# Etschbeijer/GibbsSampling

Hardware: NVIDIA B200
Metric: gibbs_window_scores_per_sec (higher is better)
Workload: dtype f64

## Files before the change

### gibbssampling_b200/csrc/gibbs_cluster.cuh

```cuda
#pragma once
#include "gibbs_kernels.cuh"

namespace gibbs {

constexpr int CL_T = 16;

__device__ __forceinline__ uint32_t cluster_ctarank() {
    uint32_t r;
    asm volatile("mov.u32 %0, %%cluster_ctarank;" : "=r"(r));
    return r;
}
__device__ __forceinline__ void cluster_barrier() {
    asm volatile("barrier.cluster.arrive.release.aligned;\n\tbarrier.cluster.wait.acquire.aligned;" ::: "memory");
}
__device__ __forceinline__ uint32_t map_to_rank(const void *smem_ptr, uint32_t rank) {
    uint32_t out;
    asm volatile("mapa.shared::cluster.u32 %0, %1, %2;" : "=r"(out) : "r"(smem_u32(smem_ptr)), "r"(rank));
    return out;
}
__device__ __forceinline__ void st_cluster_u32(uint32_t addr, uint32_t v) {
    asm volatile("st.shared::cluster.u32 [%0], %1;" ::"r"(addr), "r"(v) : "memory");
}
__device__ __forceinline__ void st_cluster_u64(uint32_t addr, uint64_t v) {
    asm volatile("st.shared::cluster.u64 [%0], %1;" ::"r"(addr), "l"(v) : "memory");
}
__device__ __forceinline__ void cp_async16(void *dst, const void *src) {
    asm volatile("cp.async.cg.shared.global [%0], [%1], 16;" ::"r"(smem_u32(dst)), "l"(src) : "memory");
}
__device__ __forceinline__ void cp_async_wait_all() { asm volatile("cp.async.commit_group;\n\tcp.async.wait_group 0;" ::: "memory"); }

template <int C>
__host__ __device__ constexpr int cl_flags_off() { return 704; }
template <int C>
__host__ __device__ constexpr int cl_delta_off() { return cl_flags_off<C>() + 2 * C * CL_T * 4; }
template <int C>
__host__ __device__ constexpr int cl_ctl_off() { return cl_delta_off<C>() + 2 * C * CL_T * 16; }
template <int C>
__host__ __device__ constexpr int cl_tables_off() { return (cl_ctl_off<C>() + 16 + 63) / 64 * 64; }
template <int C>
__host__ __device__ inline size_t cluster_smem_bytes(int n, int row_words) {
    return (size_t)cl_tables_off<C>() + (size_t)CL_T * WARP_TABLE_BYTES + (size_t)CL_T * 2 * row_words * 4 + (size_t)n * 4 * sizeof(WEnt);
}

template <int KP, int C>
static __global__ void __launch_bounds__(32 * CL_T, 1) chain_cluster_kernel(const ChainArgs a) {
    extern __shared__ __align__(128) unsigned char smem_raw[];
    constexpr int T = CL_T, THREADS = 32 * CL_T, GW = C * CL_T;
    const int tid = threadIdx.x, lane = tid & 31, warp = tid >> 5;
    const uint32_t crank = cluster_ctarank();
    const int gw = (int)crank * T + warp;
    const int entry = blockIdx.x / C;
    if (entry >= *a.pending_in_n) return;
    const int chain = a.pending_in[entry];

    const int N = a.s.n, k = a.k, row_words = a.s.row_words;
    int32_t *total = reinterpret_cast<int32_t *>(smem_raw);
    int32_t *fix = reinterpret_cast<int32_t *>(smem_raw + 512);
    uint32_t *lut = reinterpret_cast<uint32_t *>(smem_raw + 640);
    int32_t *flags = reinterpret_cast<int32_t *>(smem_raw + cl_flags_off<C>());
    uint64_t *delta = reinterpret_cast<uint64_t *>(smem_raw + cl_delta_off<C>());
    int32_t *ctl = reinterpret_cast<int32_t *>(smem_raw + cl_ctl_off<C>());
    WarpTables WT;
    {
        unsigned char *b = smem_raw + cl_tables_off<C>() + warp * WARP_TABLE_BYTES;
        WT.wcol = reinterpret_cast<double *>(b);
        WT.ptab = reinterpret_cast<int32_t *>(b + 1024);
        WT.lgcol = reinterpret_cast<int32_t *>(b + 2048);
        WT.counts = reinterpret_cast<int32_t *>(b + 2560);
    }
    require_aligned_tables(WT);
    uint32_t *rows = reinterpret_cast<uint32_t *>(smem_raw + cl_tables_off<C>() + T * WARP_TABLE_BYTES) + warp * 2 * row_words;
    WEnt *wtab_s = reinterpret_cast<WEnt *>(smem_raw + cl_tables_off<C>() + T * WARP_TABLE_BYTES + (size_t)T * 2 * row_words * 4);

    int32_t *sites = a.sites + (size_t)chain * N;
    double *hv = a.hv + (size_t)chain * N;
    double *scores = a.scores + (size_t)chain * N;

    if (tid < 16) lut[tid] = hist_lut_entry(tid);
    {
        const int4 *src = reinterpret_cast<const int4 *>(a.wtab);
        int4 *dst = reinterpret_cast<int4 *>(wtab_s);
        for (int i = tid; i < N * 4; i += THREADS) dst[i] = __ldg(src + i);
    }
    uint32_t r_flag = 0, r_delta = 0;
    if (lane < C) {
        r_flag = map_to_rank(flags + gw, (uint32_t)lane);
        r_delta = map_to_rank(delta + 2 * gw, (uint32_t)lane);
    }
    __syncthreads();
    cluster_barrier();

    unsigned long long st_updates = 0, st_windows = 0, st_slow = 0, st_spec = 0;
    int st_sweeps = 0, capped = 0;
    int phase, sweeps_in_phase;
    {
        const int r = a.resume[chain];
        phase = r & 127;
        capped = (r >> 7) & 1;
        sweeps_in_phase = r >> 8;
    }
    bool resumed = true, paused = false;
    const int ulen = a.s.uniform_len;

    auto fetch_row = [&](int seq, int slot) {
        const uint4 *src = reinterpret_cast<const uint4 *>(a.s.packed + (size_t)seq * row_words);
        uint4 *dst = reinterpret_cast<uint4 *>(rows + slot * row_words);
        for (int i = lane; i < (row_words >> 2); i += 32) cp_async16(dst + i, src + i);
    };

    while (phase != PH_DONE) {
        const int mode = phase == PH_LEFT ? SHIFT_LEFT : phase == PH_RIGHT ? SHIFT_RIGHT : SHIFT_NONE;
        if (phase == PH_LEFT || phase == PH_RIGHT || (phase == PH_GREEDY && (sweeps_in_phase == 0 || resumed)))
            site_counts<KP, T>(a.s, sites, -1, k, mode, total, lut, fix, tid);
        resumed = false;
        bool changed = false;
        int n0 = 0;
        int width = (phase == PH_GREEDY) ? max(1, min(GW, a.min_width)) : GW;
        unsigned round = 0;
        int have = -1, have_slot = 0;
        int pf_n = -1, pf_site = 0, pf_len = 0;
        double pf_hv = 0.0;
        {
            const int n = n0 + gw;
            if (n < N) {
                fetch_row(n, 0);
                have = n;
                have_slot = 0;
                pf_n = n;
                pf_site = __ldcg(sites + n);
                pf_hv = __ldcg(hv + n);
                pf_len = ulen > 0 ? ulen : __ldg(a.s.len + n);
            }
        }
        while (n0 < N) {
            const int n = n0 + gw;
            const bool active = n < N && gw < width;
            int flag = 0, w = 0, Wn = 0;
            double p = 0.0;
            uint64_t own = 0, neu = 0;
            const int n_pred = n + GW;
            if (n < N) {
                if (have != n) {
                    cp_async_wait_all();
                    __syncwarp();
                    fetch_row(n, have_slot);
                    have = n;
                }
                cp_async_wait_all();
                __syncwarp();
            }
            const int cur_slot = have_slot;
            int nx_site = 0, nx_len = 0;
            double nx_hv = 0.0;
            if (n_pred < N) {
                fetch_row(n_pred, cur_slot ^ 1);
                nx_site = __ldcg(sites + n_pred);
                nx_hv = __ldcg(hv + n_pred);
                nx_len = ulen > 0 ? ulen : __ldg(a.s.len + n_pred);
            }
            int site_n = 0;
            if (active) {
                const uint32_t *row = rows + cur_slot * row_words;
                int len_n;
                double hv_n;
                if (pf_n == n) {
                    site_n = pf_site;
                    hv_n = pf_hv;
                    len_n = pf_len;
                } else {
                    site_n = __ldcg(sites + n);
                    hv_n = __ldcg(hv + n);
                    len_n = ulen > 0 ? ulen : __ldg(a.s.len + n);
                }
                Wn = len_n - k + 1;
                own = kmer_shared<KP>(row, shifted_site(site_n, len_n, k, mode));
                build_tables_impl<KP, false, true>(WT, total, true, own, k, wtab_s, lane, 0);
                const bool slow = pick_argmax<KP>(WT, row, Wn, k, a.fast_ok, lane, p, w);
                const bool accept = score_improves(p, hv_n, hv_n != hv_n ? __ldcg(scores + n) : 0.0);
                const bool moved = accept && (w != site_n);
                if (moved && phase == PH_GREEDY) neu = kmer_shared<KP>(row, w);
                flag = (accept ? 1 : 0) | (moved ? 2 : 0) | (slow ? 4 : 0) | 8;
            }
            const uint32_t par = (round & 1u);
            ++round;
            if (lane < C) {
                if ((flag & 2) && phase == PH_GREEDY) {
                    st_cluster_u64(r_delta + par * GW * 16, own);
                    st_cluster_u64(r_delta + par * GW * 16 + 8, neu);
                }
                st_cluster_u32(r_flag + par * GW * 4, (uint32_t)flag);
            }
            cluster_barrier();
            const int32_t *fl = flags + par * GW;
            unsigned movers_lo = __ballot_sync(FULL, lane < GW && (fl[lane < GW ? lane : 0] & 2) != 0);
            unsigned movers_hi[(GW + 31) / 32] = {};
            movers_hi[0] = movers_lo;
#pragma unroll
            for (int q = 1; q < (GW + 31) / 32; ++q) movers_hi[q] = __ballot_sync(FULL, (fl[q * 32 + lane] & 2) != 0);
            int first_mover = GW;
            bool any_moved = false;
#pragma unroll
            for (int q = (GW + 31) / 32 - 1; q >= 0; --q)
                if (movers_hi[q]) {
                    any_moved = true;
                    first_mover = q * 32 + __ffs(movers_hi[q]) - 1;
                }
            if (phase != PH_GREEDY) first_mover = GW;
            const int last_commit = min(first_mover, width - 1);
            changed |= any_moved;
            if (active) {
                if (gw <= last_commit) {
                    st_updates += 1;
                    st_windows += (unsigned long long)Wn;
                    st_slow += (flag & 4) ? 1 : 0;
                    if ((flag & 1) && lane == 0) {
                        sites[n] = w;
                        hv[n] = p;
                    }
                } else {
                    st_spec += 1;
                }
            }
            const int committed = min(last_commit + 1, N - n0);
            n0 += committed;
            if (phase == PH_GREEDY) {
                if (first_mover < GW) {
                    if (warp == 0 && lane < k) {
                        const uint64_t o = delta[(par * GW + first_mover) * 2], nw = delta[(par * GW + first_mover) * 2 + 1];
                        const int bo = (int)((o >> (2 * lane)) & 3u), bn = (int)((nw >> (2 * lane)) & 3u);
                        if (bo != bn) {
                            total[lane * 4 + bo] -= 1;
                            total[lane * 4 + bn] += 1;
                        }
                    }
                    __syncthreads();
                    width = max(max(1, min(GW, a.min_width)), width >> 1);
                } else {
                    width = min(GW, width * 2);
                }
            }
            if (n_pred < N) {
                if (committed == GW) {
                    have = n_pred;
                    have_slot = cur_slot ^ 1;
                    pf_n = n_pred;
                    pf_site = nx_site;
                    pf_hv = nx_hv;
                    pf_len = nx_len;
                } else {
                    have = -2;
                    have_slot = cur_slot;
                    pf_n = -1;
                }
            } else {
                have = -2;
                have_slot = cur_slot;
                pf_n = -1;
            }
        }
        cp_async_wait_all();
        __syncwarp();
        st_sweeps += 1;
        ++sweeps_in_phase;
        bool next = !changed;
        if (!next && sweeps_in_phase >= a.max_sweeps) {
            next = true;
            capped = 1;
        }
        if (next) {
            sweeps_in_phase = 0;
            phase = next_phase(phase + 1, a.phase_mask);
        }
        int want_pause = 0;
        if (phase != PH_DONE && a.pause_below > 0 && crank == 0 && tid == 0)
            want_pause = (*(volatile int32_t *)a.active <= a.pause_below) ? 1 : 0;
// ... 41 lines not shown
```

### gibbssampling_b200/csrc/gibbs_device.cuh

```cuda
#pragma once
#include <cuda_runtime.h>
#include <stdint.h>
#include <type_traits>

namespace gibbs {

constexpr unsigned FULL = 0xffffffffu;
constexpr int LG_FRAC_BITS = 11;
constexpr int KEY_IDX_BITS = 8;
constexpr int MAX_COLS = 32;
constexpr double LN2 = 0.6931471805599453;

enum ShiftMode { SHIFT_NONE = 0, SHIFT_LEFT = 1, SHIFT_RIGHT = 2 };
enum StatSlot { ST_SITE_UPDATES = 0, ST_WINDOW_SCORES = 1, ST_SWEEPS = 2, ST_EXACT_RESCANS = 3, ST_CAPPED = 4,
                ST_SPECULATED = 5, ST_NSLOTS = 8 };

struct __align__(16) WEnt {
    double w;
    int32_t lg;
    int32_t pad;
};

struct DeviceSeqs {
    const uint32_t *packed;
// ... 328 lines not shown
                        if (2 * p + 1 < k) dst[e1] += v1;
                    } else {
                        atomicAdd(&dst[e0], v0);
                        if (2 * p + 1 < k) atomicAdd(&dst[e1], v1);
                    }
                }
            }
            lo[p] = hi[p] = 0;
        }
    }
};

template <int KP>
struct KmerCounter {
    static constexpr int NW = (KP > 8) ? 2 : 1;
    static constexpr bool HI4 = (KP == 9 || KP == 10);
    using Word = typename std::conditional<(KP > 8), uint64_t, uint32_t>::type;
    uint32_t nib[HI4 ? 1 : NW][3][2];
    uint32_t byt[NW][3][2][2];
    uint32_t hq[HI4 ? 3 : 1];
    int quads;
    __device__ __forceinline__ void clear() {
#pragma unroll
        for (int w = 0; w < NW; ++w)
#pragma unroll
            for (int b = 0; b < 3; ++b)
#pragma unroll
                for (int p = 0; p < 2; ++p) {
                    if (!HI4 || w == 0) nib[HI4 ? 0 : w][b][p] = 0;
                    byt[w][b][p][0] = byt[w][b][p][1] = 0;
                }
        if (HI4) hq[0] = hq[1] = hq[2] = 0;
        quads = 0;
    }
    __device__ __forceinline__ void spill() {
#pragma unroll
        for (int w = 0; w < NW; ++w)
#pragma unroll
            for (int b = 0; b < 3; ++b)
#pragma unroll
                for (int p = 0; p < 2; ++p) {
                    uint32_t v;
                    if (HI4 && w == 1) {
                        v = (p == 0 ? hq[b] : (hq[b] >> 2)) & 0x33333333u;
                    } else {
                        v = nib[HI4 ? 0 : w][b][p];
                        nib[HI4 ? 0 : w][b][p] = 0;
                    }
                    byt[w][b][p][0] += v & 0x0F0F0F0Fu;
                    byt[w][b][p][1] += (v >> 4) & 0x0F0F0F0Fu;
                }
        if (HI4) hq[0] = hq[1] = hq[2] = 0;
        quads = 0;
    }
    __device__ __forceinline__ void add4(const Word x[4]) {
        if (quads == 3) spill();
#pragma unroll
        for (int w = 0; w < (HI4 ? 1 : NW); ++w) {
            uint32_t f[4][3];
#pragma unroll
            for (int i = 0; i < 4; ++i) {
                const uint32_t v = (uint32_t)(x[i] >> (32 * w)), t = v >> 1;
                f[i][0] = v & ~t & 0x55555555u;
                f[i][1] = ~v & t & 0x55555555u;
                f[i][2] = v & t & 0x55555555u;
            }
#pragma unroll
            for (int b = 0; b < 3; ++b) {
                const uint32_t s3 = f[0][b] + f[1][b] + f[2][b];
                nib[w][b][0] += (s3 & 0x33333333u) + (f[3][b] & 0x11111111u);
                nib[w][b][1] += ((s3 >> 2) & 0x33333333u) + ((f[3][b] >> 2) & 0x11111111u);
            }
        }
        if constexpr (HI4) {
            const uint32_t h01 = __byte_perm((uint32_t)((uint64_t)x[0] >> 32), (uint32_t)((uint64_t)x[1] >> 32), 0x0040);
            const uint32_t h23 = __byte_perm((uint32_t)((uint64_t)x[2] >> 32), (uint32_t)((uint64_t)x[3] >> 32), 0x0040);
            const uint32_t v = __byte_perm(h01, h23, 0x5410), t = v >> 1;
            hq[0] += v & ~t & 0x55555555u;
            hq[1] += ~v & t & 0x55555555u;
            hq[2] += v & t & 0x55555555u;
        }
        ++quads;
    }
    __device__ __forceinline__ void flush(int32_t *dst, int k, int added, bool first, int lane) {
        spill();
        uint32_t mine[NW] = {};
#pragma unroll
        for (int w = 0; w < NW; ++w)
#pragma unroll
            for (int b = 0; b < 3; ++b)
#pragma unroll
                for (int p = 0; p < 2; ++p)
#pragma unroll
                    for (int h = 0; h < 2; ++h)
#pragma unroll
                        for (int g = 0; g < 2; ++g) {
                            const int it = (((b * 2 + p) * 2 + h) * 2 + g);
                            const int col0 = (HI4 && w == 1) ? 16 + 2 * h + p : 16 * w + 4 * g + 2 * h + p;
                            if (col0 < 2 * KP) {
                                const uint32_t s = __reduce_add_sync(FULL, (byt[w][b][p][h] >> (8 * g)) & 0x00FF00FFu);
                                if (lane == it) mine[w] = s;
                            }
                        }
        {
            const int g = lane & 1, h = (lane >> 1) & 1, p = (lane >> 2) & 1, b = lane >> 3;
#pragma unroll
            for (int w = 0; w < NW; ++w) {
                const int32_t v0 = (int32_t)(mine[w] & 0xFFFFu), v1 = (int32_t)(mine[w] >> 16);
                if (HI4 && w == 1) {
                    const int32_t half = v0 + v1, tot = half + __shfl_xor_sync(FULL, half, 1);
                    const int c = 16 + 2 * h + p;
                    if (lane < 24 && g == 0 && c < k) dst[c * 4 + b + 1] = first ? tot : dst[c * 4 + b + 1] + tot;
                } else if (lane < 24) {
                    const int c0 = 16 * w + 4 * g + 2 * h + p, c1 = c0 + 8;
                    if (c0 < k) dst[c0 * 4 + b + 1] = first ? v0 : dst[c0 * 4 + b + 1] + v0;
                    if (c1 < k) dst[c1 * 4 + b + 1] = first ? v1 : dst[c1 * 4 + b + 1] + v1;
                }
            }
        }
#pragma unroll
        for (int w = 0; w < NW; ++w)
#pragma unroll
            for (int b = 0; b < 3; ++b)
#pragma unroll
                for (int p = 0; p < 2; ++p) byt[w][b][p][0] = byt[w][b][p][1] = 0;
        if (lane < k) dst[lane * 4] = first ? added : dst[lane * 4] + added;
        __syncwarp();
    }
    static __device__ __forceinline__ void finish(int32_t *dst, int k, int lane) {
        if (lane < k) dst[lane * 4] -= dst[lane * 4 + 1] + dst[lane * 4 + 2] + dst[lane * 4 + 3];
        __syncwarp();
    }
};

template <int KP, bool SROWS>
__device__ __forceinline__ typename KmerCounter<KP>::Word gather_kmer(const uint32_t *__restrict__ rows, int row_words, int i, int pos) {
    uint32_t w0, w1, w2 = 0;
    if (SROWS) {
        const uint32_t *p = rows + (i * row_words + (pos >> 4));
        w0 = p[0];
        w1 = p[1];
        if (KP > 8) w2 = p[2];
    } else {
        const uint32_t *p = rows + (size_t)i * row_words + (pos >> 4);
        w0 = __ldg(p);
        w1 = __ldg(p + 1);
        if (KP > 8) w2 = __ldg(p + 2);
    }
    const uint32_t lo = __funnelshift_r(w0, w1, 2 * pos);
    if constexpr (KP > 8) {
        return ((uint64_t)__funnelshift_r(w1, w2, 2 * pos) << 32) | lo;
    } else {
        return lo;
    }
}
template <int KP>
__device__ __forceinline__ typename KmerCounter<KP>::Word gather_kmer_wide(const uint64_t *__restrict__ wide, int wide_words, int i, int pos) {
    const uint64_t v = __ldg(wide + (size_t)i * wide_words + (pos >> 3)) >> (2 * (pos & 7));
    return (typename KmerCounter<KP>::Word)v;
}

template <int KP, int T>
__device__ __forceinline__ void site_counts(const DeviceSeqs &s, const int32_t *sites, int exclude, int k, int mode,
                                            int32_t *total, const uint32_t *lut, int32_t *fix, int tid) {
    constexpr int THREADS = 32 * T;
    for (int e = tid; e < MAX_COLS * 4; e += THREADS) total[e] = 0;
    if (s.mask != nullptr && tid < MAX_COLS) fix[tid] = 0;
    team_sync<T>();
    Hist<KP> h;
    h.clear();
    const int iters = (s.n + THREADS - 1) / THREADS;
    for (int it0 = 0; it0 < iters; it0 += 255) {
        const int it1 = min(iters, it0 + 255);
        for (int it = it0; it < it1; ++it) {
            const int i = it * THREADS + tid;
            h.maybe_spill(1);
            if (i < s.n && i != exclude) {
                const int site = __ldcg(sites + i);
                if (site >= 0) {
                    const int pos = shifted_site(site, __ldg(s.len + i), k, mode);
                    h.add(kmer_global<KP>(s.packed + (size_t)i * s.row_words, pos), lut);
                    if (row_masked(s, i)) hist_fix(s.mask, s.row_words, i, pos, k, fix);
                }
            }
        }
        h.template flush_add<(T > 1)>(total, k, tid & 31);
// ... 50 lines not shown

template <int OFF>
__device__ __forceinline__ double lds_f64(uint32_t addr) {
    double v;
    asm volatile("ld.shared.f64 %0, [%1+%2];" : "=d"(v) : "r"(addr), "n"(OFF));
    return v;
}
template <int KP, int J>
struct WindowProduct {
    static __device__ __forceinline__ double upto(uint32_t lo, uint32_t hi, uint32_t wcol_addr, int k) {
        const double prev = WindowProduct<KP, J - 1>::upto(lo, hi, wcol_addr, k);
        constexpr int c = J - 1;
        const uint32_t word = c < 16 ? lo : hi;
        constexpr int sh = 2 * (c & 15);
        const uint32_t off = (sh >= 3 ? (word >> (sh - 3)) : (word << (3 - sh))) & 24u;
        const double f = lds_f64<c * 32>(off | wcol_addr);
        return c < k ? __dmul_rn(prev, f) : prev;
    }
};
template <int KP>
struct WindowProduct<KP, 0> {
    static __device__ __forceinline__ double upto(uint32_t, uint32_t, uint32_t, int) { return 1.0; }
};

template <int KP>
__device__ __forceinline__ double exact_window(const uint32_t *row, int w, int k, const double *wcol) {
    const uint64_t kmer = kmer_shared<KP>(row, w);
    return WindowProduct<KP, 2 * KP>::upto((uint32_t)kmer, (uint32_t)(kmer >> 32), smem_u32(wcol), k);
}

__device__ __forceinline__ bool better(double ohv, int ow, double hv, int w) { return ohv > hv || (ohv == hv && ow < w); }

__device__ __forceinline__ void warp_argmax(double &hv, int &w) {
#pragma unroll
    for (int o = 16; o; o >>= 1) {
        const double ohv = __shfl_xor_sync(FULL, hv, o);
        const int ow = __shfl_xor_sync(FULL, w, o);
        if (better(ohv, ow, hv, w)) {
            hv = ohv;
            w = ow;
        }
    }
}

template <int KP>
__device__ __forceinline__ void scan_exact_all(const uint32_t *row, int W, int k, const double *wcol, int lane,
                                               double &hv_out, int &w_out) {
    double hv = 0.0;
    int hw = 0;
    for (int w = lane; w < W; w += 32) {
        const double p = exact_window<KP>(row, w, k, wcol);
        if (p > hv) {
            hv = p;
            hw = w;
        }
    }
    warp_argmax(hv, hw);
    hv_out = hv;
    w_out = hw;
}

template <int KP>
__device__ __noinline__ void scan_exact_masked(const uint32_t *row, const uint32_t *__restrict__ mask, int row_words, int n,
                                               int W, int k, const double *wcol, int lane, double &hv_out, int &w_out) {
    double hv = 0.0;
    int hw = 0;
    for (int w = lane; w < W; w += 32) {
        if (mask_kmer(mask, row_words, n, w, k) != 0) continue;
        const double p = exact_window<KP>(row, w, k, wcol);
        if (p > hv) {
            hv = p;
            hw = w;
        }
    }
    warp_argmax(hv, hw);
    hv_out = hv;
    w_out = hw;
}

template <int OFF>
__device__ __forceinline__ int32_t lds_ptab(uint32_t addr) {
    int32_t v;
    asm volatile("ld.shared.s32 %0, [%1+%2];" : "=r"(v) : "r"(addr), "n"(OFF));
    return v;
}
template <int KP, int P>
struct PairSum {
    static __device__ __forceinline__ int32_t of(const uint32_t *ad, int e) {
        return lds_ptab<P * 64>(ad[e + P]) + PairSum<KP, P + 1>::of(ad, e);
    }
};
template <int KP>
struct PairSum<KP, KP> {
    static __device__ __forceinline__ int32_t of(const uint32_t *, int) { return 0; }
};

template <int KP, int CH, bool MASK>
__device__ __forceinline__ int32_t score_chunk(const uint32_t *a, const uint32_t *b, uint32_t ptab_addr, int idx, int lim) {
    constexpr int NE = CH / 2 + KP - 1;
    uint32_t adE[NE], adO[NE];
#pragma unroll
    for (int t = 0; t < NE; ++t) {
        const int j = t & 7;
        const uint32_t xe = a[t >> 3], xo = b[t >> 3];
        adE[t] = ((j == 0 ? (xe << 2) : (xe >> (4 * j - 2))) & 0x3cu) | ptab_addr;
        adO[t] = ((j == 0 ? (xo << 2) : (xo >> (4 * j - 2))) & 0x3cu) | ptab_addr;
    }
    int32_t key[CH];
#pragma unroll
    for (int i = 0; i < CH; ++i) {
        const int e = i >> 1;
        int32_t v = idx + ((i & 1) ? PairSum<KP, 0>::of(adO, e) : PairSum<KP, 0>::of(adE, e));
        if (MASK) v = (i < lim) ? v : INT32_MIN;
        key[i] = v;
    }
#pragma unroll
    for (int st = 1; st < CH; st *= 2)
#pragma unroll
        for (int i = 0; i + st < CH; i += 2 * st) key[i] = max(key[i], key[i + st]);
    return key[0];
}

template <int KP, int CH>
struct ScanGeom {
    static constexpr int NB = CH + 2 * KP - 1;
    static constexpr int NWA = (NB + 15) / 16;
    static constexpr int RPS = 256;
    static constexpr int CPS = 32 * RPS;
};

template <int CH>
__device__ __forceinline__ int chunk_base(int c, int W) { return max(0, min(c * CH, W - CH)); }

template <int KP, int CH>
__device__ __forceinline__ void scan_fast(const uint32_t *row, int W, const int32_t *ptab, int lane, int32_t &M1,
                                          int32_t &M2, int &S1) {
    using G = ScanGeom<KP, CH>;
    const int n_chunks = (W + CH - 1) / CH;
    const uint32_t ptab_addr = smem_u32(ptab);
    M1 = INT32_MIN;
    M2 = INT32_MIN;
    S1 = 0;
    for (int seg = 0, c0 = 0; c0 < n_chunks; ++seg, c0 += G::CPS) {
        const int c_end = min(n_chunks, c0 + G::CPS);
        int idx = 255;
        for (int c = c0 + lane; c < c_end; c += 32, --idx) {
            const int base0 = chunk_base<CH>(c, W);
            const uint32_t *p = row + (base0 >> 4);
            const int sh = (base0 & 15) * 2;
            uint32_t raw[G::NWA + 1], a[G::NWA + 1], b[G::NWA];
#pragma unroll
            for (int i = 0; i <= G::NWA; ++i) raw[i] = p[i];
#pragma unroll
            for (int i = 0; i < G::NWA; ++i) a[i] = __funnelshift_r(raw[i], raw[i + 1], sh);
            a[G::NWA] = 0;
#pragma unroll
            for (int i = 0; i < G::NWA; ++i) b[i] = __funnelshift_r(a[i], a[i + 1], 2);
            int32_t cm;
            if (W >= CH) cm = score_chunk<KP, CH, false>(a, b, ptab_addr, idx, CH);
            else cm = score_chunk<KP, CH, true>(a, b, ptab_addr, idx, W);
            if (cm > M1) {
                M2 = max(M2, M1);
                M1 = cm;
                S1 = seg;
            } else {
                M2 = max(M2, cm);
// ... 76 lines not shown
```

### gibbssampling_b200/csrc/gibbs_init_tu.cu

```cuda
#include "gibbs_kernels.cuh"

#if !defined(GIBBS_INIT_TU_KIND)
#error "compile with -DGIBBS_INIT_TU_KIND=0|1|2|3 (see _build.py)"
#endif

namespace gibbs {

#if GIBBS_INIT_TU_KIND == 3
template <int KPV>
static cudaError_t launch_tiled_one(const ChainArgs &a, int grid, int smem, cudaStream_t stream, int tile_rows) {
    auto kernel = init_tiled_kernel<KPV>;
    if (smem > 48 * 1024) {
        const cudaError_t e = cudaFuncSetAttribute(kernel, cudaFuncAttributeMaxDynamicSharedMemorySize, smem);
        if (e != cudaSuccess) return e;
    }
    kernel<<<grid, TILED_WARPS * 32, smem, stream>>>(a, tile_rows, philox_round_keys(a.seed));
    return cudaGetLastError();
}

cudaError_t launch_init_tiled(const ChainArgs &a, int grid, int smem, cudaStream_t stream, int tile_rows) {
    switch ((a.k + 1) / 2) {
#define X(KPV) case KPV: return launch_tiled_one<KPV>(a, grid, smem, stream, tile_rows);
        X(1) X(2) X(3) X(4) X(5) X(6) X(7) X(8) X(9) X(10) X(11) X(12) X(13) X(14) X(15) X(16)
#undef X
    default: return cudaErrorInvalidValue;
    }
}
#else
template <int KPV>
static cudaError_t launch_one(const ChainArgs &a, int grid, int smem, cudaStream_t stream) {
#if GIBBS_INIT_TU_KIND == 2
    auto kernel = init_smem_kernel<KPV>;
    constexpr int threads = ISM_WARPS * 32;
#else
    auto kernel = init_kernel<KPV, GIBBS_INIT_TU_KIND == 1>;
    constexpr int threads = INIT_WARPS * 32;
#endif
    if (smem > 48 * 1024) {
        const cudaError_t e = cudaFuncSetAttribute(kernel, cudaFuncAttributeMaxDynamicSharedMemorySize, smem);
        if (e != cudaSuccess) return e;
    }
    kernel<<<grid, threads, smem, stream>>>(a);
    return cudaGetLastError();
}

#if GIBBS_INIT_TU_KIND == 0
#define GIBBS_INIT_TU_NAME launch_init_wide
#elif GIBBS_INIT_TU_KIND == 1
#define GIBBS_INIT_TU_NAME launch_init_wide_drift
#else
#define GIBBS_INIT_TU_NAME launch_init_smem
#endif

cudaError_t GIBBS_INIT_TU_NAME(const ChainArgs &a, int grid, int smem, cudaStream_t stream) {
    switch ((a.k + 1) / 2) {
#define X(KPV) case KPV: return launch_one<KPV>(a, grid, smem, stream);
        X(1) X(2) X(3) X(4) X(5) X(6) X(7) X(8) X(9) X(10) X(11) X(12) X(13) X(14) X(15) X(16)
#undef X
    default: return cudaErrorInvalidValue;
    }
}
#endif

}
```

### gibbssampling_b200/csrc/gibbs_kernels.cuh

```cuda
#pragma once
#include "gibbs_device.cuh"
#include "gibbs_drift_dev.cuh"

namespace gibbs {

enum Phase { PH_INIT = 0, PH_GREEDY = 1, PH_LEFT = 2, PH_RIGHT = 3, PH_DONE = 4 };

__device__ __forceinline__ int next_phase(int from, int mask) {
    int ph = from;
    while (ph < PH_DONE && !((mask >> ph) & 1)) ++ph;
    return ph;
}

static __global__ void pack_kernel(const uint8_t *__restrict__ ascii, const int64_t *__restrict__ off, int n, int row_words,
                            uint32_t *__restrict__ packed, uint32_t *__restrict__ mask, int32_t *__restrict__ rowflag,
                            int32_t *__restrict__ len_out, int *flags) {
    const int64_t t = (int64_t)blockIdx.x * blockDim.x + threadIdx.x;
    if (t >= (int64_t)n * row_words) return;
    const int i = (int)(t / row_words), wd = (int)(t % row_words);
    const int64_t o = off[i];
    const int len = (int)(off[i + 1] - o);
    if (wd == 0) len_out[i] = len;
    uint32_t v = 0, m = 0;
    int other = 0;
// ... 6 lines not shown
            uint32_t code = 0;
            if (c == 'A') code = 0;
            else if (c == 'C') code = 1;
            else if (c == 'G') code = 2;
            else if (c == 'T') code = 3;
            else if (c >= 42 && c <= 90) {
                m |= 3u << (2 * x);
                ++other;
                if (c == '-') atomicExch(flags + 2, 1);
            } else {
                atomicExch(flags, 1 + (int)c);
            }
            v |= code << (2 * x);
        }
    }
    packed[t] = v;
    mask[t] = m;
    if (other) {
        atomicAdd(flags + 1, other);
        rowflag[i] = 1;
    }
}

static __global__ void wide_kernel(const uint32_t *__restrict__ packed, int n, int row_words, int wide_words, uint64_t *__restrict__ wide) {
    const int64_t t = (int64_t)blockIdx.x * blockDim.x + threadIdx.x;
    if (t >= (int64_t)n * wide_words) return;
    const int i = (int)(t / wide_words), m = (int)(t % wide_words);
    const uint32_t *row = packed + (size_t)i * row_words;
    const int w = m >> 1;
    uint32_t a = row[w], b = w + 1 < row_words ? row[w + 1] : 0u, c = w + 2 < row_words ? row[w + 2] : 0u;
    uint64_t v = ((uint64_t)b << 32) | a;
    if (m & 1) v = (v >> 16) | ((uint64_t)c << 48);
    wide[t] = v;
}

static __global__ void wtab_kernel(int n, double pc, double den, double q0, double q1, double q2, double q3, WEnt *wtab,
                            int *range) {
    const int t = blockIdx.x * blockDim.x + threadIdx.x;
    if (t >= n * 4) return;
    const int c = t >> 2, b = t & 3;
    const double q = b == 0 ? q0 : b == 1 ? q1 : b == 2 ? q2 : q3;
    const double w = __ddiv_rn(__ddiv_rn(__dadd_rn((double)c, pc), den), q);
    WEnt e;
    e.w = w;
    e.pad = 0;
    const bool normal = (w >= 2.2250738585072014e-308) && (w <= 1.7976931348623157e308);
    if (normal) {
        double units = rint(log2(w) * (double)(1 << LG_FRAC_BITS));
        units = fmin(fmax(units, -4000000.0), 4000000.0);
        const int u = (int)units;
        e.lg = u * (1 << KEY_IDX_BITS);
        atomicMin(&range[0], u);
        atomicMax(&range[1], u);
    } else {
        e.lg = 0;
        atomicExch(&range[2], 1);
    }
    wtab[t] = e;
}

#ifndef GIBBS_P0_NB_CHAIN
#define GIBBS_P0_NB_CHAIN 1
#endif
#ifndef GIBBS_P0_NB_INIT_SMALL
#define GIBBS_P0_NB_INIT_SMALL 4
#endif
#ifndef GIBBS_P0_NB_INIT_LARGE
#define GIBBS_P0_NB_INIT_LARGE 2
#endif
#ifndef GIBBS_T4_MIN_BLOCKS
#define GIBBS_T4_MIN_BLOCKS 7
#endif
#ifndef GIBBS_T8_MIN_BLOCKS
#define GIBBS_T8_MIN_BLOCKS 3
#endif
#ifndef GIBBS_T16_MIN_BLOCKS
#define GIBBS_T16_MIN_BLOCKS 1
#endif
#ifndef GIBBS_INIT_MIN_BLOCKS
#define GIBBS_INIT_MIN_BLOCKS 2
#endif
template <int KP, int NB, bool MASKED, bool SROWS, bool UNI, bool PHILOX, bool WIDE = false>
__device__ __forceinline__ void random_draw_loop(const ChainArgs &a, uint64_t chain_uid, int chain_local, int n, int32_t *counts,
                                                 int lane, int32_t *fix, const uint32_t *base_rows) {
    using Word = typename KmerCounter<KP>::Word;
    const int N = a.s.n, k = a.k;
    const int row_words = a.s.row_words;
    const uint64_t base = (uint64_t)n * (uint64_t)(N - 1);
    const uint64_t d_end = base + (uint64_t)(N - 1);
    const uint64_t blk0 = base >> 2, blk1 = (d_end + 3) >> 2;
    const int n_blk = (int)(blk1 - blk0);
    const int iters = (n_blk + 32 * NB - 1) / (32 * NB);
    const int r_first = (int)((int64_t)(blk0 << 2) - (int64_t)base);
    const uint32_t range_u = (uint32_t)(a.s.uniform_len - k + 1);
    KmerCounter<KP> h;
    h.clear();
    constexpr int FLUSH_ROUNDS = 63 / NB;
    bool first = true;
    for (int it0 = 0; it0 < iters; it0 += FLUSH_ROUNDS) {
        const int it1 = min(iters, it0 + FLUSH_ROUNDS);
        for (int it = it0; it < it1; ++it) {
            Word kmer[NB][4];
#pragma unroll
            for (int q = 0; q < NB; ++q) {
                const int bi = (it * NB + q) * 32 + lane;
                uint32_t wd[4] = {0, 0, 0, 0};
                if (PHILOX) {
                    const uint64_t blk = blk0 + (uint64_t)bi;
                    const uint4 r = philox4x32_10(make_uint4((uint32_t)blk, (uint32_t)(blk >> 32), (uint32_t)chain_uid, (uint32_t)(chain_uid >> 32)),
                                                  make_uint2((uint32_t)a.seed, (uint32_t)(a.seed >> 32)));
                    wd[0] = r.x; wd[1] = r.y; wd[2] = r.z; wd[3] = r.w;
                }
                const int r0 = r_first + 4 * bi;
#pragma unroll
                for (int x = 0; x < 4; ++x) {
                    const bool ok = (unsigned)(r0 + x) < (unsigned)(N - 1);
                    const int r = ok ? r0 + x : 0;
                    const int i = r + (r >= n ? 1 : 0);
                    const uint32_t range = UNI ? range_u : (uint32_t)(__ldg(a.s.len + i) - k + 1);
                    int pos;
                    if (PHILOX) {
                        pos = (int)__umulhi(wd[x], range);
                    } else {
                        const int64_t d = (int64_t)base + r;
                        const double u = d < a.uniforms_per_chain ? __ldg(a.uniforms + (size_t)chain_local * a.uniforms_per_chain + d)
                                                                  : 0.0;
                        pos = (int)(u * (double)range);
                        pos = min(max(pos, 0), (int)range - 1);
                    }
                    const Word km = WIDE ? gather_kmer_wide<KP>(a.s.wide, a.s.wide_words, i, pos) : gather_kmer<KP, SROWS>(base_rows, row_words, i, pos);
                    kmer[q][x] = ok ? km : (Word)0;
                    if (MASKED && ok && __ldg(a.s.rowflag + i) != 0) hist_fix(a.s.mask, row_words, i, pos, k, fix);
                }
            }
#pragma unroll
            for (int q = 0; q < NB; ++q) h.add4(kmer[q]);
        }
        h.flush(counts, k, it1 == iters ? N - 1 : 0, first, lane);
        first = false;
    }
    KmerCounter<KP>::finish(counts, k, lane);
}

template <int KP, int NB, bool MASKED, bool SROWS = false>
__device__ __forceinline__ void random_loo_counts_impl(const ChainArgs &a, uint64_t chain_uid, int chain_local, int n,
                                                       int32_t *counts, int lane, int32_t *fix,
                                                       const uint32_t *rows = nullptr) {
    const int N = a.s.n, k = a.k;
    if (MASKED) fix[lane] = 0;
    if (N < 2) {
        for (int e = lane; e < 8 * KP; e += 32) counts[e] = 0;
        __syncwarp();
        return;
    }
    const uint32_t *const base_rows = SROWS ? rows : a.s.packed;
    bool done = false;
    if constexpr (!SROWS && KP <= 13) {
        if (a.rng_mode == 0 && a.s.wide != nullptr && k <= 25) {
            if (a.s.uniform_len > 0) random_draw_loop<KP, NB, MASKED, false, true, true, true>(a, chain_uid, chain_local, n, counts, lane, fix, base_rows);
            else random_draw_loop<KP, NB, MASKED, false, false, true, true>(a, chain_uid, chain_local, n, counts, lane, fix, base_rows);
            done = true;
        }
    }
    if (done) {
    } else if (a.rng_mode != 0) random_draw_loop<KP, 1, MASKED, SROWS, false, false>(a, chain_uid, chain_local, n, counts, lane, fix, base_rows);
    else if (a.s.uniform_len > 0) random_draw_loop<KP, NB, MASKED, SROWS, true, true>(a, chain_uid, chain_local, n, counts, lane, fix, base_rows);
    else random_draw_loop<KP, NB, MASKED, SROWS, false, true>(a, chain_uid, chain_local, n, counts, lane, fix, base_rows);
    if (MASKED) {
        if (lane < k) counts[lane * 4] -= fix[lane];
        __syncwarp();
    }
}

template <int KP, bool MASKED>
static __device__ __noinline__ void random_loo_counts_call(const ChainArgs &a, uint64_t chain_uid, int chain_local, int n,
                                                           int32_t *counts, int lane, int32_t *fix) {
    random_loo_counts_impl<KP, GIBBS_P0_NB_CHAIN, MASKED>(a, chain_uid, chain_local, n, counts, lane, fix);
}

constexpr int INIT_WARPS = 8;

__host__ __device__ inline int init_smem_bytes(int row_words) {
    return 64 + INIT_WARPS * 16 + INIT_WARPS * WARP_TABLE_BYTES + INIT_WARPS * 2 * row_words * 4;
}

template <int KP, bool DRIFT = false>
static __global__ void __launch_bounds__(INIT_WARPS * 32, GIBBS_INIT_MIN_BLOCKS) init_kernel(const ChainArgs a) {
    extern __shared__ __align__(128) unsigned char smem_raw[];
    const int tid = threadIdx.x, lane = tid & 31, warp = tid >> 5;
    const int N = a.s.n, k = a.k, row_words = a.s.row_words;
    uint32_t *lut = reinterpret_cast<uint32_t *>(smem_raw);
    uint64_t *bar = reinterpret_cast<uint64_t *>(smem_raw + 64) + warp * 2;
    WarpTables WT;
    {
        unsigned char *b = smem_raw + 64 + INIT_WARPS * 16 + warp * WARP_TABLE_BYTES;
        WT.wcol = reinterpret_cast<double *>(b);
        WT.ptab = reinterpret_cast<int32_t *>(b + 1024);
        WT.lgcol = reinterpret_cast<int32_t *>(b + 2048);
        WT.counts = reinterpret_cast<int32_t *>(b + 2560);
    }
    require_aligned_tables(WT);
    uint32_t *rows = reinterpret_cast<uint32_t *>(smem_raw + 64 + INIT_WARPS * 16 + INIT_WARPS * WARP_TABLE_BYTES) +
                     warp * 2 * row_words;
    if (tid < 16) lut[tid] = hist_lut_entry(tid);
    if (lane == 0) {
        mbar_init(bar, 1);
        mbar_init(bar + 1, 1);
        fence_barrier_init();
    }
    __syncthreads();

    const long long total = (long long)a.n_chains * N;
    const long long stride = (long long)gridDim.x * INIT_WARPS;
    long long item = (long long)blockIdx.x * INIT_WARPS + warp;
    const uint32_t bytes = (uint32_t)row_words * 4u;
    auto issue = [&](long long it, uint32_t v) {
        if (lane == 0) {
            const int slot = (int)(v & 1u);
            mbar_expect_tx(bar + slot, bytes);
            bulk_g2s(rows + slot * row_words, a.s.packed + (size_t)(it % N) * row_words, bytes, bar + slot);
        }
    };
    unsigned long long st_updates = 0, st_windows = 0, st_slow = 0;
    uint32_t v = 0;
    if (item < total) issue(item, 0);
    while (item < total) {
        const long long next = item + stride;
        if (next < total) issue(next, v + 1);
        mbar_wait(bar + (v & 1u), (v >> 1) & 1u);
        const uint32_t *row = rows + (v & 1u) * row_words;
        const int chain = (int)(item / N), n = (int)(item % N);
        const int Wn = __ldg(a.s.len + n) - k + 1;
        random_loo_counts_impl<KP, (KP <= 6 ? GIBBS_P0_NB_INIT_SMALL : GIBBS_P0_NB_INIT_LARGE), false>(a, (uint64_t)a.chain_id_base + (uint64_t)chain, chain, n, WT.counts, lane, WT.lgcol);
        double p;
        int w;
        bool slow;
        if constexpr (DRIFT) {
            int f0[4], cn[4];
            const bool given = a.ppm_given != nullptr;
            const bool fast = a.drift_fast_ok && !given;
            drift_tables<KP>(WT, WT.counts, false, 0, k, a, given, fast, n, lane, f0, cn);
            slow = drift_pick<KP>(WT, row, Wn, k, a, fast, f0, cn, lane, p, w, -1, n);
        } else {
            build_tables<KP>(WT, WT.counts, false, 0, k, a.wtab, lane);
            slow = pick_argmax<KP>(WT, row, Wn, k, a.fast_ok, lane, p, w);
        }
        if (lane == 0) {
            a.sites[(size_t)chain * N + n] = w;
            a.hv[(size_t)chain * N + n] = p;
        }
        st_updates += 1;
        st_windows += (unsigned long long)Wn;
        st_slow += slow ? 1 : 0;
        __syncwarp();
        item = next;
        ++v;
    }
    if (lane == 0) {
        atomicAdd(a.stats + ST_SITE_UPDATES, st_updates);
        atomicAdd(a.stats + ST_WINDOW_SCORES, st_windows);
        atomicAdd(a.stats + ST_EXACT_RESCANS, st_slow);
    }
    if (blockIdx.x == 0 && tid == 0) atomicAdd(a.stats + ST_SWEEPS, (unsigned long long)a.n_chains);
}

#ifndef GIBBS_ISM_WARPS
#define GIBBS_ISM_WARPS 24
#endif
#ifndef GIBBS_P0_NB_ISM
#define GIBBS_P0_NB_ISM 1
#endif
constexpr int ISM_WARPS = GIBBS_ISM_WARPS;

__host__ __device__ constexpr int ism_table_bytes(int kp) { return 192 * kp; }
__host__ __device__ inline size_t init_smem_rows_bytes(int n, int row_words) { return ((size_t)n * row_words * 4 + 63) / 64 * 64; }
__host__ __device__ inline size_t init_smem_total_bytes(int n, int row_words, int kp) {
    return init_smem_rows_bytes(n, row_words) + (size_t)ISM_WARPS * ism_table_bytes(kp);
}

template <int KP>
static __global__ void __launch_bounds__(ISM_WARPS * 32, 1) init_smem_kernel(const ChainArgs a) {
    extern __shared__ __align__(128) unsigned char smem_raw[];
    const int tid = threadIdx.x, lane = tid & 31, warp = tid >> 5;
    const int N = a.s.n, k = a.k, row_words = a.s.row_words;
    uint32_t *rows = reinterpret_cast<uint32_t *>(smem_raw);
    WarpTables WT;
    {
        unsigned char *b = smem_raw + init_smem_rows_bytes(N, row_words) + warp * ism_table_bytes(KP);
        WT.wcol = reinterpret_cast<double *>(b);
        WT.ptab = reinterpret_cast<int32_t *>(b + 64 * KP);
        WT.lgcol = reinterpret_cast<int32_t *>(b + 128 * KP);
        WT.counts = reinterpret_cast<int32_t *>(b + 160 * KP);
    }
    require_aligned_tables(WT);
    {
        const uint4 *src = reinterpret_cast<const uint4 *>(a.s.packed);
        uint4 *dst = reinterpret_cast<uint4 *>(rows);
        const int n16 = N * (row_words >> 2);
        for (int i = tid; i < n16; i += ISM_WARPS * 32) dst[i] = __ldg(src + i);
    }
    __syncthreads();
    const long long total = (long long)a.n_chains * N;
    const long long stride = (long long)gridDim.x * ISM_WARPS;
    unsigned long long st_updates = 0, st_windows = 0, st_slow = 0;
    for (long long item = (long long)blockIdx.x * ISM_WARPS + warp; item < total; item += stride) {
        const int chain = (int)(item / N), n = (int)(item % N);
        const int Wn = __ldg(a.s.len + n) - k + 1;
        random_loo_counts_impl<KP, GIBBS_P0_NB_ISM, false, true>(a, (uint64_t)a.chain_id_base + (uint64_t)chain, chain, n, WT.counts,
                                                                 lane, WT.lgcol, rows);
        build_tables<KP>(WT, WT.counts, false, 0, k, a.wtab, lane);
        double p;
        int w;
        const bool slow = pick_argmax<KP>(WT, rows + (size_t)n * row_words, Wn, k, a.fast_ok, lane, p, w);
        if (lane == 0) {
            a.sites[(size_t)chain * N + n] = w;
            a.hv[(size_t)chain * N + n] = p;
        }
        st_updates += 1;
        st_windows += (unsigned long long)Wn;
        st_slow += slow ? 1 : 0;
        __syncwarp();
    }
    if (lane == 0) {
        atomicAdd(a.stats + ST_SITE_UPDATES, st_updates);
        atomicAdd(a.stats + ST_WINDOW_SCORES, st_windows);
        atomicAdd(a.stats + ST_EXACT_RESCANS, st_slow);
    }
    if (blockIdx.x == 0 && tid == 0) atomicAdd(a.stats + ST_SWEEPS, (unsigned long long)a.n_chains);
}

#ifndef GIBBS_TILED_WARPS
#define GIBBS_TILED_WARPS 16
#endif
constexpr int TILED_WARPS = GIBBS_TILED_WARPS;
#ifndef GIBBS_TILED_NB
#define GIBBS_TILED_NB 1
#endif

template <int KP, bool UNI>
__device__ __forceinline__ void tile_draws(const ChainArgs &a, const PhiloxKeys &pk, uint64_t chain_uid, uint64_t base, int n, int ra,
                                           int rb, int i0, const uint32_t *tile, uint32_t range_u, KmerCounter<KP> &h, int &since,
                                           bool &first, int32_t *counts, int lane) {
    using Word = typename KmerCounter<KP>::Word;
    const int k = a.k, row_words = a.s.row_words;
    const uint64_t blkA = (base + (uint64_t)ra) >> 2, blkB = (base + (uint64_t)rb + 3) >> 2;
    const int n_blk = (int)(blkB - blkA);
    constexpr int NB = GIBBS_TILED_NB;
    const int iters = (n_blk + 32 * NB - 1) / (32 * NB);
    const int r_first = (int)((int64_t)(blkA << 2) - (int64_t)base);
    const unsigned span = (unsigned)(rb - ra);
    const int lo_blk = r_first == ra ? 0 : 1;
    const int hi_blk = (rb - r_first) >> 2;
    const int hole_off = n - r_first;
    const int hole_blk = (hole_off > 0 && (hole_off & 3) != 0) ? (hole_off >> 2) : -1;
    for (int it = 0; it < iters; ++it) {
        int r0[NB];
        bool act[NB];
#pragma unroll
        for (int q = 0; q < NB; ++q) {
            const int bi = (it * NB + q) * 32 + lane;
            r0[q] = r_first + 4 * bi;
            act[q] = bi < n_blk;
        }
        const int b_first = it * NB * 32, b_last = b_first + NB * 32;
        const bool plain = b_first >= lo_blk && (b_last <= hi_blk || hi_blk == n_blk) && !(hole_blk >= b_first && hole_blk < b_last);
        Word kmer[NB][4];
        if (plain) {
#pragma unroll
            for (int q = 0; q < NB; ++q) {
#pragma unroll
                for (int x = 0; x < 4; ++x) kmer[q][x] = 0;
                if (act[q]) {
                    const uint64_t blk = blkA + (uint64_t)((it * NB + q) * 32 + lane);
                    const uint4 r4 = philox4x32_10_keyed(make_uint4((uint32_t)blk, (uint32_t)(blk >> 32), (uint32_t)chain_uid, (uint32_t)(chain_uid >> 32)), pk);
                    const uint32_t wd[4] = {r4.x, r4.y, r4.z, r4.w};
                    const int ib = r0[q] + (r0[q] >= n ? 1 : 0) - i0;
#pragma unroll
                    for (int x = 0; x < 4; ++x) {
                        const uint32_t range = UNI ? range_u : (uint32_t)(__ldg(a.s.len + i0 + ib + x) - k + 1);
                        const int pos = (int)__umulhi(wd[x], range);
                        kmer[q][x] = gather_kmer<KP, true>(tile, row_words, ib + x, pos);
                    }
                }
            }
        } else {
#pragma unroll
            for (int q = 0; q < NB; ++q) {
                const uint64_t blk = blkA + (uint64_t)((it * NB + q) * 32 + lane);
                const uint4 r4 = philox4x32_10_keyed(make_uint4((uint32_t)blk, (uint32_t)(blk >> 32), (uint32_t)chain_uid, (uint32_t)(chain_uid >> 32)), pk);
                const uint32_t wd[4] = {r4.x, r4.y, r4.z, r4.w};
#pragma unroll
                for (int x = 0; x < 4; ++x) {
// ... 285 lines not shown
```

Measured before the change: 443.8 billion.

## Replace per-round cluster barrier with st.async and mbarrier transaction counting

Each warp's per-round flag and delta exchange across the cluster now uses st.async stores that complete transaction bytes on a double-buffered mbarrier in each destination CTA. Consumers wait on the mbarrier phase instead of a full cluster-wide arrive/wait barrier. Deltas are always written, so the byte count is fixed per round. The round counter now persists across phases so the parity stays consistent. This removes a full cluster barrier per round but adds mbarrier bookkeeping. Buffer reuse safety now depends on the double buffering, since no barrier separates a round's reads from the next writes to the same slot.

```diff
diff --git a/gibbssampling_b200/csrc/gibbs_cluster.cuh b/gibbssampling_b200/csrc/gibbs_cluster.cuh
--- a/gibbssampling_b200/csrc/gibbs_cluster.cuh
+++ b/gibbssampling_b200/csrc/gibbs_cluster.cuh
@@ -21,8 +21,25 @@
 __device__ __forceinline__ void st_cluster_u32(uint32_t addr, uint32_t v) {
     asm volatile("st.shared::cluster.u32 [%0], %1;" ::"r"(addr), "r"(v) : "memory");
 }
-__device__ __forceinline__ void st_cluster_u64(uint32_t addr, uint64_t v) {
-    asm volatile("st.shared::cluster.u64 [%0], %1;" ::"r"(addr), "l"(v) : "memory");
+__device__ __forceinline__ void st_async_u32(uint32_t addr, uint32_t v, uint32_t mbar) {
+    asm volatile("st.async.shared::cluster.mbarrier::complete_tx::bytes.u32 [%0], %1, [%2];" ::"r"(addr), "r"(v), "r"(mbar) : "memory");
+}
+__device__ __forceinline__ void st_async_v2u64(uint32_t addr, uint64_t v0, uint64_t v1, uint32_t mbar) {
+    asm volatile("st.async.shared::cluster.mbarrier::complete_tx::bytes.v2.u64 [%0], {%1, %2}, [%3];" ::"r"(addr), "l"(v0), "l"(v1),
+                 "r"(mbar) : "memory");
+}
+__device__ __forceinline__ void mbar_init(uint64_t *bar, uint32_t count) {
+    asm volatile("mbarrier.init.shared::cta.b64 [%0], %1;" ::"r"(smem_u32(bar)), "r"(count) : "memory");
+}
+__device__ __forceinline__ void mbar_arrive_expect_tx(uint64_t *bar, uint32_t bytes) {
+    asm volatile("mbarrier.arrive.expect_tx.shared::cta.b64 _, [%0], %1;" ::"r"(smem_u32(bar)), "r"(bytes) : "memory");
+}
+__device__ __forceinline__ void mbar_wait_parity(uint64_t *bar, uint32_t parity) {
+    uint32_t done;
+    do {
+        asm volatile("{\n\t.reg .pred p;\n\tmbarrier.try_wait.parity.acquire.cta.shared::cta.b64 p, [%1], %2;\n\tselp.u32 %0, 1, 0, p;\n\t}"
+                     : "=r"(done) : "r"(smem_u32(bar)), "r"(parity) : "memory");
+    } while (!done);
 }
 __device__ __forceinline__ void cp_async16(void *dst, const void *src) {
     asm volatile("cp.async.cg.shared.global [%0], [%1], 16;" ::"r"(smem_u32(dst)), "l"(src) : "memory");
@@ -36,7 +53,9 @@
 template <int C>
 __host__ __device__ constexpr int cl_ctl_off() { return cl_delta_off<C>() + 2 * C * CL_T * 16; }
 template <int C>
-__host__ __device__ constexpr int cl_tables_off() { return (cl_ctl_off<C>() + 16 + 63) / 64 * 64; }
+__host__ __device__ constexpr int cl_mbar_off() { return cl_ctl_off<C>() + 16; }
+template <int C>
+__host__ __device__ constexpr int cl_tables_off() { return (cl_mbar_off<C>() + 16 + 63) / 64 * 64; }
 template <int C>
 __host__ __device__ inline size_t cluster_smem_bytes(int n, int row_words) {
     return (size_t)cl_tables_off<C>() + (size_t)CL_T * WARP_TABLE_BYTES + (size_t)CL_T * 2 * row_words * 4 + (size_t)n * 4 * sizeof(WEnt);
@@ -60,6 +79,7 @@
     int32_t *flags = reinterpret_cast<int32_t *>(smem_raw + cl_flags_off<C>());
     uint64_t *delta = reinterpret_cast<uint64_t *>(smem_raw + cl_delta_off<C>());
     int32_t *ctl = reinterpret_cast<int32_t *>(smem_raw + cl_ctl_off<C>());
+    uint64_t *mbar = reinterpret_cast<uint64_t *>(smem_raw + cl_mbar_off<C>());
     WarpTables WT;
     {
         unsigned char *b = smem_raw + cl_tables_off<C>() + warp * WARP_TABLE_BYTES;
@@ -82,10 +102,16 @@
         int4 *dst = reinterpret_cast<int4 *>(wtab_s);
         for (int i = tid; i < N * 4; i += THREADS) dst[i] = __ldg(src + i);
     }
-    uint32_t r_flag = 0, r_delta = 0;
+    uint32_t r_flag = 0, r_delta = 0, r_mbar = 0;
     if (lane < C) {
         r_flag = map_to_rank(flags + gw, (uint32_t)lane);
         r_delta = map_to_rank(delta + 2 * gw, (uint32_t)lane);
+        r_mbar = map_to_rank(mbar, (uint32_t)lane);
+    }
+    if (tid == 0) {
+        mbar_init(mbar, 1);
+        mbar_init(mbar + 1, 1);
+        asm volatile("fence.mbarrier_init.release.cluster;" ::: "memory");
     }
     __syncthreads();
     cluster_barrier();
@@ -101,6 +127,7 @@
     }
     bool resumed = true, paused = false;
     const int ulen = a.s.uniform_len;
+    unsigned round = 0;
 
     auto fetch_row = [&](int seq, int slot) {
         const uint4 *src = reinterpret_cast<const uint4 *>(a.s.packed + (size_t)seq * row_words);
@@ -116,7 +143,6 @@
         bool changed = false;
         int n0 = 0;
         int width = (phase == PH_GREEDY) ? max(1, min(GW, a.min_width)) : GW;
-        unsigned round = 0;
         int have = -1, have_slot = 0;
         int pf_n = -1, pf_site = 0, pf_len = 0;
         double pf_hv = 0.0;
@@ -181,16 +207,15 @@
                 if (moved && phase == PH_GREEDY) neu = kmer_shared<KP>(row, w);
                 flag = (accept ? 1 : 0) | (moved ? 2 : 0) | (slow ? 4 : 0) | 8;
             }
-            const uint32_t par = (round & 1u);
+            constexpr uint32_t ROUND_TX = 4 + 16;
+            const uint32_t par = (round & 1u), phase_par = (round >> 1) & 1u;
             ++round;
+            if (tid == 0) mbar_arrive_expect_tx(mbar + par, GW * ROUND_TX);
             if (lane < C) {
-                if ((flag & 2) && phase == PH_GREEDY) {
-                    st_cluster_u64(r_delta + par * GW * 16, own);
-                    st_cluster_u64(r_delta + par * GW * 16 + 8, neu);
-                }
-                st_cluster_u32(r_flag + par * GW * 4, (uint32_t)flag);
-            }
-            cluster_barrier();
+                st_async_v2u64(r_delta + par * GW * 16, own, neu, r_mbar + par * 8);
+                st_async_u32(r_flag + par * GW * 4, (uint32_t)flag, r_mbar + par * 8);
+            }
+            mbar_wait_parity(mbar + par, phase_par);
             const int32_t *fl = flags + par * GW;
             unsigned movers_lo = __ballot_sync(FULL, lane < GW && (fl[lane < GW ? lane : 0] & 2) != 0);
             unsigned movers_hi[(GW + 31) / 32] = {};
```

Result: no change. 443.7 billion (median of 6 runs) (-0.0%).

## Add shared-memory uniform-length draw path with precomputed Philox keys and staged flush

Applied to the files above, without the earlier changes.

For the shared-memory init kernel with uniform-length sequences, the random k-mer draw loop now computes the Philox stream with round keys precomputed on the host, then fetches packed words straight from shared memory with inline ld.shared and a branchless row-skip walk. The row buffer gets zero-padded guard rows on both sides so clamped or overrunning reads stay in bounds without bounds checks. The k-mer histogram flush writes reduced sums through a small shared stage, filled by lane 0, instead of per-lane predicated register selects. This adds shared-memory footprint and a __syncwarp, and reuses the wcol table region as scratch space.

```diff
diff --git a/gibbssampling_b200/csrc/gibbs_device.cuh b/gibbssampling_b200/csrc/gibbs_device.cuh
--- a/gibbssampling_b200/csrc/gibbs_device.cuh
+++ b/gibbssampling_b200/csrc/gibbs_device.cuh
@@ -434,7 +434,8 @@
         }
         ++quads;
     }
-    __device__ __forceinline__ void flush(int32_t *dst, int k, int added, bool first, int lane) {
+    template <bool STAGED = false>
+    __device__ __forceinline__ void flush(int32_t *dst, int k, int added, bool first, int lane, uint32_t *stage = nullptr) {
         spill();
         uint32_t mine[NW] = {};
 #pragma unroll
@@ -451,9 +452,18 @@
                             const int col0 = (HI4 && w == 1) ? 16 + 2 * h + p : 16 * w + 4 * g + 2 * h + p;
                             if (col0 < 2 * KP) {
                                 const uint32_t s = __reduce_add_sync(FULL, (byt[w][b][p][h] >> (8 * g)) & 0x00FF00FFu);
-                                if (lane == it) mine[w] = s;
+                                if constexpr (STAGED) {
+                                    if (lane == 0) stage[24 * w + it] = s;
+                                } else if (lane == it) {
+                                    mine[w] = s;
+                                }
                             }
                         }
+        if constexpr (STAGED) {
+            __syncwarp();
+#pragma unroll
+            for (int w = 0; w < NW; ++w) mine[w] = lane < 24 ? stage[24 * w + lane] : 0u;
+        }
         {
             const int g = lane & 1, h = (lane >> 1) & 1, p = (lane >> 2) & 1, b = lane >> 3;
 #pragma unroll
@@ -670,6 +680,12 @@
 __device__ __forceinline__ int32_t lds_ptab(uint32_t addr) {
     int32_t v;
     asm volatile("ld.shared.s32 %0, [%1+%2];" : "=r"(v) : "r"(addr), "n"(OFF));
+    return v;
+}
+template <int OFF>
+__device__ __forceinline__ uint32_t lds_u32(uint32_t addr) {
+    uint32_t v;
+    asm volatile("ld.shared.u32 %0, [%1+%2];" : "=r"(v) : "r"(addr), "n"(OFF));
     return v;
 }
 template <int KP, int P>
diff --git a/gibbssampling_b200/csrc/gibbs_init_tu.cu b/gibbssampling_b200/csrc/gibbs_init_tu.cu
--- a/gibbssampling_b200/csrc/gibbs_init_tu.cu
+++ b/gibbssampling_b200/csrc/gibbs_init_tu.cu
@@ -40,7 +40,11 @@
         const cudaError_t e = cudaFuncSetAttribute(kernel, cudaFuncAttributeMaxDynamicSharedMemorySize, smem);
         if (e != cudaSuccess) return e;
     }
+#if GIBBS_INIT_TU_KIND == 2
+    kernel<<<grid, threads, smem, stream>>>(a, philox_round_keys(a.seed));
+#else
     kernel<<<grid, threads, smem, stream>>>(a);
+#endif
     return cudaGetLastError();
 }
 
diff --git a/gibbssampling_b200/csrc/gibbs_kernels.cuh b/gibbssampling_b200/csrc/gibbs_kernels.cuh
--- a/gibbssampling_b200/csrc/gibbs_kernels.cuh
+++ b/gibbssampling_b200/csrc/gibbs_kernels.cuh
@@ -112,8 +112,9 @@
 #endif
 template <int KP, int NB, bool MASKED, bool SROWS, bool UNI, bool PHILOX, bool WIDE = false>
 __device__ __forceinline__ void random_draw_loop(const ChainArgs &a, uint64_t chain_uid, int chain_local, int n, int32_t *counts,
-                                                 int lane, int32_t *fix, const uint32_t *base_rows) {
+                                                 int lane, int32_t *fix, const uint32_t *base_rows, const PhiloxKeys *pk = nullptr) {
     using Word = typename KmerCounter<KP>::Word;
+    constexpr bool SMEM_UNI = SROWS && UNI && PHILOX;
     const int N = a.s.n, k = a.k;
     const int row_words = a.s.row_words;
     const uint64_t base = (uint64_t)n * (uint64_t)(N - 1);
@@ -131,6 +132,29 @@
         const int it1 = min(iters, it0 + FLUSH_ROUNDS);
         for (int it = it0; it < it1; ++it) {
             Word kmer[NB][4];
+            if constexpr (SMEM_UNI) {
+                const uint32_t S = (uint32_t)row_words * 4u, rows_addr = smem_u32(base_rows);
+#pragma unroll
+                for (int q = 0; q < NB; ++q) {
+                    const int bi = (it * NB + q) * 32 + lane;
+                    const uint64_t blk = blk0 + (uint64_t)bi;
+                    const uint4 r = philox4x32_10_keyed(make_uint4((uint32_t)blk, (uint32_t)(blk >> 32), (uint32_t)chain_uid, (uint32_t)(chain_uid >> 32)), *pk);
+                    const uint32_t wd[4] = {r.x, r.y, r.z, r.w};
+                    const int r0 = min(r_first + 4 * bi, N - 1);
+                    const int hx = n - r0;
+                    uint32_t ra = rows_addr + (uint32_t)(r0 + (hx <= 0 ? 1 : 0)) * S;
+#pragma unroll
+                    for (int x = 0; x < 4; ++x) {
+                        if (x > 0) ra += hx == x ? 2 * S : S;
+                        const uint32_t pos = __umulhi(wd[x], range_u);
+                        const uint32_t p = ra + ((pos >> 4) << 2);
+                        const uint32_t w0 = lds_u32<0>(p), w1 = lds_u32<4>(p);
+                        const uint32_t lo = __funnelshift_r(w0, w1, 2 * pos);
+                        if constexpr (KP > 8) kmer[q][x] = ((uint64_t)__funnelshift_r(w1, lds_u32<8>(p), 2 * pos) << 32) | lo;
+                        else kmer[q][x] = lo;
+                    }
+                }
+            } else {
 #pragma unroll
             for (int q = 0; q < NB; ++q) {
                 const int bi = (it * NB + q) * 32 + lane;
@@ -163,10 +187,11 @@
                     if (MASKED && ok && __ldg(a.s.rowflag + i) != 0) hist_fix(a.s.mask, row_words, i, pos, k, fix);
                 }
             }
+            }
 #pragma unroll
             for (int q = 0; q < NB; ++q) h.add4(kmer[q]);
         }
-        h.flush(counts, k, it1 == iters ? N - 1 : 0, first, lane);
+        h.template flush<SMEM_UNI>(counts, k, it1 == iters ? N - 1 : 0, first, lane, reinterpret_cast<uint32_t *>(fix));
         first = false;
     }
     KmerCounter<KP>::finish(counts, k, lane);
@@ -175,7 +200,7 @@
 template <int KP, int NB, bool MASKED, bool SROWS = false>
 __device__ __forceinline__ void random_loo_counts_impl(const ChainArgs &a, uint64_t chain_uid, int chain_local, int n,
                                                        int32_t *counts, int lane, int32_t *fix,
-                                                       const uint32_t *rows = nullptr) {
+                                                       const uint32_t *rows = nullptr, const PhiloxKeys *pk = nullptr) {
     const int N = a.s.n, k = a.k;
     if (MASKED) fix[lane] = 0;
     if (N < 2) {
@@ -194,7 +219,7 @@
     }
     if (done) {
     } else if (a.rng_mode != 0) random_draw_loop<KP, 1, MASKED, SROWS, false, false>(a, chain_uid, chain_local, n, counts, lane, fix, base_rows);
-    else if (a.s.uniform_len > 0) random_draw_loop<KP, NB, MASKED, SROWS, true, true>(a, chain_uid, chain_local, n, counts, lane, fix, base_rows);
+    else if (a.s.uniform_len > 0) random_draw_loop<KP, NB, MASKED, SROWS, true, true>(a, chain_uid, chain_local, n, counts, lane, fix, base_rows, pk);
     else random_draw_loop<KP, NB, MASKED, SROWS, false, true>(a, chain_uid, chain_local, n, counts, lane, fix, base_rows);
     if (MASKED) {
         if (lane < k) counts[lane * 4] -= fix[lane];
@@ -303,17 +328,17 @@
 constexpr int ISM_WARPS = GIBBS_ISM_WARPS;
 
 __host__ __device__ constexpr int ism_table_bytes(int kp) { return 192 * kp; }
-__host__ __device__ inline size_t init_smem_rows_bytes(int n, int row_words) { return ((size_t)n * row_words * 4 + 63) / 64 * 64; }
+__host__ __device__ inline size_t init_smem_rows_bytes(int n, int row_words) { return ((size_t)(n + 7) * row_words * 4 + 63) / 64 * 64; }
 __host__ __device__ inline size_t init_smem_total_bytes(int n, int row_words, int kp) {
     return init_smem_rows_bytes(n, row_words) + (size_t)ISM_WARPS * ism_table_bytes(kp);
 }
 
 template <int KP>
-static __global__ void __launch_bounds__(ISM_WARPS * 32, 1) init_smem_kernel(const ChainArgs a) {
+static __global__ void __launch_bounds__(ISM_WARPS * 32, 1) init_smem_kernel(const ChainArgs a, const PhiloxKeys pk) {
     extern __shared__ __align__(128) unsigned char smem_raw[];
     const int tid = threadIdx.x, lane = tid & 31, warp = tid >> 5;
     const int N = a.s.n, k = a.k, row_words = a.s.row_words;
-    uint32_t *rows = reinterpret_cast<uint32_t *>(smem_raw);
+    uint32_t *rows = reinterpret_cast<uint32_t *>(smem_raw) + 3 * row_words;
     WarpTables WT;
     {
         unsigned char *b = smem_raw + init_smem_rows_bytes(N, row_words) + warp * ism_table_bytes(KP);
@@ -325,9 +350,9 @@
     require_aligned_tables(WT);
     {
         const uint4 *src = reinterpret_cast<const uint4 *>(a.s.packed);
-        uint4 *dst = reinterpret_cast<uint4 *>(rows);
-        const int n16 = N * (row_words >> 2);
-        for (int i = tid; i < n16; i += ISM_WARPS * 32) dst[i] = __ldg(src + i);
+        uint4 *dst = reinterpret_cast<uint4 *>(smem_raw);
+        const int r16 = row_words >> 2, lo = 3 * r16, hi = (N + 3) * r16, n16 = (N + 7) * r16;
+        for (int i = tid; i < n16; i += ISM_WARPS * 32) dst[i] = (i >= lo && i < hi) ? __ldg(src + (i - lo)) : make_uint4(0, 0, 0, 0);
     }
     __syncthreads();
     const long long total = (long long)a.n_chains * N;
@@ -337,7 +362,7 @@
         const int chain = (int)(item / N), n = (int)(item % N);
         const int Wn = __ldg(a.s.len + n) - k + 1;
         random_loo_counts_impl<KP, GIBBS_P0_NB_ISM, false, true>(a, (uint64_t)a.chain_id_base + (uint64_t)chain, chain, n, WT.counts,
-                                                                 lane, WT.lgcol, rows);
+                                                                 lane, reinterpret_cast<int32_t *>(WT.wcol), rows, &pk);
         build_tables<KP>(WT, WT.counts, false, 0, k, a.wtab, lane);
         double p;
         int w;
```

Result: faster. 444.1 billion before, 448.9 billion after (median of 6 runs) (+1.1%).
